# chris-chambers/deap

Hardware: AMD Instinct MI355X
Metric: GPop/s (node-evals×cases/s) symreg 64K pop×1M cases, 1/2/4/8 GPUs (higher is better)
Workload: dtype f64

## Files before the change

### deap_amd/_lib.py

```python
import ctypes
import os

import numpy as np

_HERE = os.path.dirname(os.path.abspath(__file__))
LIB_PATH = os.environ.get("DEAP_AMD_LIB") or os.path.join(_HERE, "libgpeval.so")

GPE_MACHINE_F = 0
GPE_MACHINE_B = 1
GPE_MODE_MSE = 0
GPE_MODE_HITS_BOOL = 1
GPE_MODE_HITS_BITS = 2
GPE_MODE_SSE_NUMPY = 3
GPE_MODE_SSE_SEQ = 4
GPE_PREC_F64 = 0
GPE_PREC_F32 = 1
GPE_NO_ERROR = 0xFFFFFFFFFFFFFFFF
GPE_ERR_VALUE = 1
GPE_ERR_OVERFLOW = 2
GPE_ERR_XINT_RANGE = 3
GPE_XINT_WORDS = 34
GPE_FLAG_NONFINITE_TERM = 1
GPE_FLAG_NAN_TERM = 2
GPE_FLAG_INF_TERM = 4
# ... 628 lines not shown
                         "asm_deep_P", "asm_deep_groups",
                         "asm_deep_waves_per_block", "redo_exact_cpp",
                         "asm_typed", "asm_typed_P", "asm_typed_groups",
                         "typed_const"),
                        list(g)))

    LAUNCHES = ("asm_fast", "asm_deep", "typed", "cpp_fast", "cpp_deep",
                "fasm", "dasm")

    def trig_classes(self, picked=False):
        if picked:
            g = (ctypes.c_int64 * len(TRIG_PICKED))()
            self._check(self.lib.gpe_last_trig_picked(self.h, g),
                        "gpe_last_trig_picked")
            return dict(zip(TRIG_PICKED, (int(v) for v in g)))
        g = (ctypes.c_int64 * 3)()
        self._check(self.lib.gpe_last_trig_classes(self.h, g),
                    "gpe_last_trig_classes")
        return dict(zip(TRIG_CLASSES, (int(v) for v in g)))

    def launch_shape(self, which):
        if isinstance(which, str):
            which = self.LAUNCHES.index(which)
        g = (ctypes.c_int64 * 12)()
        self._check(self.lib.gpe_last_launch_shape(self.h, int(which), g, 12),
                    "gpe_last_launch_shape")
        return dict(zip(("programs", "P", "wpb", "waves", "n_slots", "K",
                         "sdepth", "n_tiles", "tiles_per_group", "groups",
                         "dbuf", "lds_bytes"), list(g)))
```

### deap_amd/csrc/asm_kernels.h

```cpp
#pragma once
namespace {

struct AsmTask {
  const uint32_t* code;
  const uint32_t* start;
  const int32_t* slot_prog;
  int64_t n_slots;
  int P;
  const double* X;
  int nv;
  const double* terms;
  int nt;
  int64_t n_cases;
  int64_t n_tiles;
  int tiles_per_group;
  double* part;
  double* case_out;
  unsigned long long* first_err;
  uint32_t* flags;
  uint32_t* redo;
  uint32_t* redo_count;
  uint64_t* redo_list;
  uint32_t redo_list_cap;
  const double* cst;
  const float* cst32;
  int diag;
  uint32_t redo_hi;
  uint32_t* base_probe;
  int dbuf;
};

constexpr int kTrigLdsDoubles = asmcore::kTrigEntries * 2 + 4;
constexpr uint32_t kTrigLdsBytes = kTrigLdsDoubles * sizeof(double);
static_assert(kTrigLdsBytes % 16 == 0, "the X tile is read with 16-byte alignment");
constexpr int kCstTable = 16;

#if GP_ASM_LOOP
#define GP_CORE_LOOPED(CODE, PROBE, PROBE_OUT, J, NMINE, DONE, RHI, LEAN, VSTART,  \
                       VTS, VACC)                                             \
  asm volatile(GP_ASM_CORE                                                  \
               : GP_ASM_T_OUTPUTS, GP_ASM_VRED_OUTPUT, GP_ASM_VINF_OUTPUT,  \
                 [jio] "+s"(J)                                              \
               : [cst] "s"(cst), [xa] "v"(xa),                              \
                 [mg] "v"(asmcore::kAsmMagic), [ps2] "v"(asmcore::kAsmPs2), \
                 [pc2] "v"(asmcore::kAsmPc2), [one] "v"(0x3ff00000u),        \
                 [probe] "s"(PROBE), [probe_out] "s"(PROBE_OUT),            \
                 [code_lo] "s"((uint32_t)(CODE)),                           \
                 [code_hi] "s"((uint32_t)((uint64_t)(CODE) >> 32)),         \
                 [nmine] "s"(NMINE), [done] "s"(DONE), [rhi] "s"(RHI),      \
                 [lean] "s"(LEAN), [vstart] "v"(VSTART), [vts] "v"(VTS),    \
                 [vacc] "v"(VACC)                                           \
               : GP_ASM_CLOBBERS)
// ... 15 lines not shown
               : GP_ASM_CLOBBERS)
#define GP_CORE_LOOPED(CODE, PROBE, PROBE_OUT, J, NMINE, DONE, RHI, LEAN, VSTART,  \
                       VTS, VACC)                                             \
  __builtin_trap()
#endif

#define GP_CORE32(PC, PROBE, PROBE_OUT)                                     \
  asm volatile(GP_ASM_CORE32                                                \
               : GP_ASM_T_OUTPUTS32                                         \
               : [pc] "s"(PC), [cst] "s"(cst), [xa] "v"(xa),               \
                 [probe] "s"(PROBE), [probe_out] "s"(PROBE_OUT)             \
               : GP_ASM_CLOBBERS32)

#define GP_CORE_DEEP(PC, PROBE, PROBE_OUT)                                  \
  asm volatile(GP_ASM_CORE_DEEP                                             \
               : GP_ASM_T_OUTPUTS_DEEP, GP_ASM_VRED_OUTPUT_DEEP, GP_ASM_VINF_OUTPUT_DEEP                   \
               : [pc] "s"(PC), [cst] "s"(cst), [xa] "v"(xa),               \
                 [mg] "v"(asmcore::kAsmMagic), [ps2] "v"(asmcore::kAsmPs2), \
                 [pc2] "v"(asmcore::kAsmPc2), [one] "v"(0x3ff00000u),        \
                 [probe] "s"(PROBE),                                        \
                 [probe_out] "s"(PROBE_OUT)                                 \
               : GP_ASM_CLOBBERS_DEEP)

#if GP_ASM_LOOP_EXACT
#define GP_CORE_EXACT_LOOPED(CODE, PROBE, PROBE_OUT, J, NMINE, DONE, RHI, LEAN,   \
                             VSTART, VTS, VACC)                               \
  asm volatile(GP_ASM_CORE_EXACT                                            \
               : GP_ASM_T_OUTPUTS_EXACT, GP_ASM_VRED_OUTPUT_EXACT,          \
                 [jio] "+s"(J)                                              \
               : [cst] "s"(cst), [xa] "v"(xa),                              \
                 [mg] "v"(asmcore::kAsmMagic), [one] "v"(0x3ff00000u),      \
                 GP_ASM_GLIBC_INPUTS_EXACT, [probe] "s"(PROBE),             \
                 [probe_out] "s"(PROBE_OUT),                                \
                 [code_lo] "s"((uint32_t)(CODE)),                           \
                 [code_hi] "s"((uint32_t)((uint64_t)(CODE) >> 32)),         \
                 [nmine] "s"(NMINE), [done] "s"(DONE), [rhi] "s"(RHI),      \
                 [lean] "s"(LEAN), [vstart] "v"(VSTART), [vts] "v"(VTS),    \
                 [vacc] "v"(VACC)                                           \
               : GP_ASM_CLOBBERS_EXACT)
#define GP_CORE_EXACT(PC, PROBE, PROBE_OUT)                                 \
  do {                                                                      \
    uint32_t j_one_ = 0;                                                    \
    GP_CORE_EXACT_LOOPED((PC), (PROBE), (PROBE_OUT), j_one_, 1u, 0u, ~0u, 0u, \
                         0u, 0u, 0u);                                       \
  } while (0)
#else
#define GP_CORE_EXACT(PC, PROBE, PROBE_OUT)                                 \
  asm volatile(GP_ASM_CORE_EXACT                                            \
               : GP_ASM_T_OUTPUTS_EXACT, GP_ASM_VRED_OUTPUT_EXACT           \
               : [pc] "s"(PC), [cst] "s"(cst), [xa] "v"(xa),               \
                 [mg] "v"(asmcore::kAsmMagic), [one] "v"(0x3ff00000u),      \
                 GP_ASM_GLIBC_INPUTS_EXACT, [probe] "s"(PROBE),             \
                 [probe_out] "s"(PROBE_OUT)                                 \
               : GP_ASM_CLOBBERS_EXACT)
#define GP_CORE_EXACT_LOOPED(CODE, PROBE, PROBE_OUT, J, NMINE, DONE, RHI, LEAN,   \
                             VSTART, VTS, VACC)                               \
  __builtin_trap()
#endif

#define GP_CORE_EXACT_DEEP(PC, PROBE, PROBE_OUT)                            \
  asm volatile(GP_ASM_CORE_EXACT_DEEP                                       \
               : GP_ASM_T_OUTPUTS_EXACT_DEEP, GP_ASM_VRED_OUTPUT_EXACT_DEEP \
               : [pc] "s"(PC), [cst] "s"(cst), [xa] "v"(xa),               \
                 [mg] "v"(asmcore::kAsmMagic), [one] "v"(0x3ff00000u),      \
                 GP_ASM_GLIBC_INPUTS_EXACT_DEEP, [probe] "s"(PROBE),        \
                 [probe_out] "s"(PROBE_OUT)                                 \
               : GP_ASM_CLOBBERS_EXACT_DEEP)

#define GP_CORE32_DEEP(PC, PROBE, PROBE_OUT)                                \
  asm volatile(GP_ASM_CORE32_DEEP                                           \
               : GP_ASM_T_OUTPUTS32_DEEP                                    \
               : [pc] "s"(PC), [cst] "s"(cst), [xa] "v"(xa),               \
                 [probe] "s"(PROBE), [probe_out] "s"(PROBE_OUT)             \
               : GP_ASM_CLOBBERS32_DEEP)

__global__ __launch_bounds__(64) void f_probe_asm(const double* cst,
                                                  uint32_t* table) {
  double T[asmcore::K];
  uint32_t vred, vinf;
// ... 207 lines not shown
  Task st{};
  st.X = a.X;
  st.nv = a.nv;
  st.terms = a.terms;
  st.nt = a.nt;
  st.n_cases = a.n_cases;
  const uint32_t ncol = (uint32_t)(a.nv + a.nt);
  auto dma_tile = [&](int64_t t, uint32_t b) {
    const uint32_t w = (uint32_t)__builtin_amdgcn_readfirstlane(wave);
    for (uint32_t col = w; col < ncol; col += (uint32_t)nwaves) {
      const double* src = (col < (uint32_t)a.nv)
                              ? a.X + (int64_t)col * a.n_cases
                              : a.terms + (int64_t)(col - a.nv) * a.n_cases;
      src += t * (K * 64) + 2 * lane;
      const uint32_t dst = kTab + b * tile_bytes + col * (uint32_t)(K * 64 * sizeof(double));
      uint32_t keep;
      asm volatile("s_mov_b32 %0, m0\n\ts_mov_b32 m0, %2\n\ts_nop 0\n\t"
                   "global_load_lds_dwordx4 %1, off\n\ts_mov_b32 m0, %0"
                   : "=&s"(keep) : "v"(src), "s"(dst) : "memory");
    }
  };
  auto tile_full = [&](int64_t t) { return (t + 1) * (K * 64) <= a.n_cases; };
  bool staged = false;
  uint32_t gflag = 0;
  for (int64_t t = t0; t < t1; ++t) {
    if (a.diag & 16) {
      uint32_t sink;
      asm volatile(".rept 40\n\tv_readlane_b32 %0, %1, 5\n\t.endr" : "=s"(sink) : "v"(lane));
    }
    if constexpr (!F32 && !EXACT) {
      done_mask |= (uint32_t)__builtin_amdgcn_ballot_w64(gflag != 0);
      gflag = my_prog >= 0 ? __hip_atomic_load(&a.redo[my_prog], __ATOMIC_RELAXED,
                                                __HIP_MEMORY_SCOPE_AGENT)
                           : 0u;
    }
    if (dbuf) {
      const uint32_t b = (uint32_t)((t - t0) & 1);
      xs = xs0 + b * tile_elems;
      ts = xs + a.nv * K * 64;
      xa = kTab + b * tile_bytes + (uint32_t)lane * (uint32_t)sizeof(R);
      vts = xa + (uint32_t)(a.nv * K * 64 * (int)sizeof(R));
      if (!staged) {
        __syncthreads();
        f_stage<K>(st, xs, t, nthreads);
        __syncthreads();
      }
      staged = t + 1 < t1 && tile_full(t + 1);
      if (staged) dma_tile(t + 1, b ^ 1u);
    } else if (!(a.diag & 2) || t == t0) {
      if (!(a.diag & 4) || t == t0) __syncthreads();
      if (!(a.diag & 8) || t == t0) f_stage<K>(st, xs, t, nthreads);
      if (!(a.diag & 4) || t == t0) __syncthreads();
    }
    const int64_t case0 = t * (K * 64) + lane;
    const bool full = (t + 1) * (K * 64) <= a.n_cases;
    auto finish = [&](int j, int prog, R (&T)[K], uint32_t (&vcase)[F32 ? K : 1],
                      uint32_t vbits, bool redo_lane) {
      if (a.diag & 1) {
        if (T[0] == R(12345) && T[1] == R(54321)) acc[lane] = vcase[0];
        return;
      }
      if (__builtin_amdgcn_ballot_w64(redo_lane)) {
        if (lane == 0) {
          const uint32_t i = atomicAdd(a.redo_count, 1u);
          if ((F32 || EXACT) && i < a.redo_list_cap)
            a.redo_list[i] = ((uint64_t)(uint32_t)prog << 32) | (uint64_t)(uint32_t)t;
          atomicOr(&a.redo[prog], 1u);
        }
        if (!F32 && !EXACT) done_mask |= 1u << j;
        return;
      }
      double hi = acc[(2 * j) * 64 + lane], lo = acc[(2 * j + 1) * 64 + lane];
      if (lean && full) {
        double s = hi, l = lo;
#pragma unroll
        for (int k = 0; k < K; ++k) {
          const double dlt = (double)T[k] - (double)ts[k * 64 + lane];
// ... 31 lines not shown
          double s, e;
          two_sum(hi, sq, s, e);
          hi = s;
          lo = lo + e;
          if (a.case_out) a.case_out[(size_t)prog * a.n_cases + c] = sq;
        }
      }
      acc[(2 * j) * 64 + lane] = hi;
      acc[(2 * j + 1) * 64 + lane] = lo;
      if (err != ~0ull) atomicMin(&a.first_err[prog], err);
      if (__builtin_amdgcn_ballot_w64(flag != 0)) {
        for (int m = 32; m >= 1; m >>= 1) flag |= __shfl_xor(flag, m, 64);
        if (lane == 0) atomicOr(&a.flags[prog], flag);
      }
    };
    if constexpr (LOOP) {
      const uint32_t lean_full = (uint32_t)__builtin_amdgcn_readfirstlane(lean && full ? 1 : 0);
      const uint32_t probe =
          (uint32_t)__builtin_amdgcn_readfirstlane(a.base_probe != nullptr ? 1 : 0);
      uint32_t* probe_out = a.base_probe;
      const double* cst = a.cst;
      const uint64_t code = (uint64_t)a.code;
      uint32_t jn = 0;
#pragma nounroll
      for (;;) {
        uint32_t jx = jn;
        const uint32_t done = (uint32_t)__builtin_amdgcn_readfirstlane(done_mask);
        R T[K];
        uint32_t vred, vinf = 0;
        if constexpr (EXACT) {
          GP_CORE_EXACT_LOOPED(code, probe, probe_out, jx, (uint32_t)n_mine, done,
                               a.redo_hi, lean_full, my_start, vts, vacc);
        } else {
          GP_CORE_LOOPED(code, probe, probe_out, jx, (uint32_t)n_mine, done, a.redo_hi,
                         lean_full, my_start, vts, vacc);
        }
        if (probe || jx >= (uint32_t)n_mine) break;
        const int prog = __builtin_amdgcn_readlane(my_prog, jx);
        uint32_t vcase[1] = {vred};
        finish((int)jx, prog, T, vcase, vinf, vred >= a.redo_hi);
        jn = jx + 1;
      }
    } else {
#pragma nounroll
      for (int j = 0; j < n_mine; ++j) {
        if (done_mask & (1u << j)) continue;
        const int prog = __builtin_amdgcn_readlane(my_prog, j);
        const uint32_t w0 = __builtin_amdgcn_readlane(my_start, j);
        const uint64_t pc = (uint64_t)(a.code + w0);
        const uint32_t probe =
            (uint32_t)__builtin_amdgcn_readfirstlane(a.base_probe != nullptr ? 1 : 0);
        uint32_t* probe_out = a.base_probe;
        R T[K];
        uint32_t vcase[F32 ? K : 1];
        uint32_t vbits = 0;
        bool redo_lane;
        if constexpr (F32) {
          const float* cst = a.cst32;
          uint32_t* vred = vcase;
          if constexpr (DEEP) {
            GP_CORE32_DEEP(pc, probe, probe_out);
          } else {
            GP_CORE32(pc, probe, probe_out);
          }
// ... 221 lines not shown
```

### deap_amd/csrc/ctx.h

```cpp
#pragma once

struct Launch {
  std::vector<int32_t> slot_prog;
  int32_t* d_slot_prog = nullptr;
  int64_t n_slots = 0;
  int P = 1;
  int sdepth = 1;
  int wpb = kWaves;
  int64_t n_tiles = 0;
  int groups = 0;
  int tiles_per_group = 0;
  int64_t waves = 0;
  double* d_part = nullptr;
  size_t part_cap = 0;
  size_t slot_cap = 0;
  int64_t programs = 0;
  int K = 0;
  bool dbuf = false;
  size_t lds = 0;
  char* h_pin = nullptr;
  size_t h_pin_cap = 0;
};


constexpr int32_t kNpAdd = -1, kNpZero = -2;
constexpr int64_t kNpChunk = 8192, kNpBlock = 128;
constexpr int kNpStack = 64;

HD double np_leaf(const double* x, int64_t n) {
  if (n < 8) {
    double res = -0.0;
    for (int64_t i = 0; i < n; ++i) res = res + x[i];
    return res;
  }
  double r[8];
  for (int j = 0; j < 8; ++j) r[j] = x[j];
  int64_t i = 8;
  for (; i < n - (n % 8); i += 8)
    for (int j = 0; j < 8; ++j) r[j] = r[j] + x[i + j];
  double res = ((r[0] + r[1]) + (r[2] + r[3])) + ((r[4] + r[5]) + (r[6] + r[7]));
  for (; i < n; ++i) res = res + x[i];
// ... 201 lines not shown
  uint64_t* d_pair_sorted = nullptr;
  size_t pair_sorted_cap = 0;
  int64_t* d_pair_off = nullptr;
  size_t pair_off_cap = 0;
  uint32_t* d_pair_nruns = nullptr;
  size_t pair_nruns_cap = 0;
  char* d_sort_tmp = nullptr;
  size_t sort_tmp_cap = 0;
  int use_asm = 1;
  int asm_pmax = 8;
  int typed_pmax = 64;
  int typed_waves = 8;
  int64_t target_blocks = 8192;
  int64_t asm_target_blocks = 65536;
  int64_t xasm_target_blocks = 65536;
  int64_t typed_target_blocks = 32768;
  int64_t min_group_tiles = 0;
  int trig_w = 14;
  int div_w = 5;
  int deal_mix = 0;
  int asm_waves = 8;
  int asm_lds_kb = 80;
  int asm_dbuf = 1;
  int lw_interleave = 1;
  int neg_fold = 1;
  int exact_all = 1;
  int trig_ranges = 2;
  std::vector<double> col_bnd;
  double* d_col_bnd = nullptr;
  unsigned long long* d_trig_cls = nullptr;
  int64_t trig_classes[8] = {0, 0, 0, 0, 0, 0, 0, 0};
  std::vector<uint32_t> debug_redo_or;
  int asm_deep_waves = 4;
  int f_waves = 8;
  int b_lanes = 1;
  int diag = 0;
  uint32_t redo_hi = (uint32_t)asmcore::LIM_HI;
  uint32_t redo_hi_deep = (uint32_t)(0x3ff + 20) << 20;
  Launch fast, deep, fasm, dasm, tasm, redo_fast, redo_deep, redo_xasm, redo_xasm_deep;
  bool last_exact_all = false;
  std::vector<int32_t> pl_fa, pl_da, pl_ta, pl_fc, pl_dc, pl_order;
  std::vector<uint32_t> pl_kc;
  uint32_t* d_kc = nullptr;
  size_t kc_cap = 0;
  int64_t n_kc = 0;
  int64_t label_true = 0;
// ... 108 lines not shown
```

### deap_amd/csrc/gen_asm.py

```python
#!/usr/bin/env python3
import os
import re
import sys

HERE = os.path.dirname(os.path.abspath(__file__))

FAMS = ["add", "sub", "rsub", "mul", "div", "rdiv", "ndiv", "nrdiv"]
FAMS_TYPED = ["add", "sub", "rsub", "mul", "div", "rdiv", "lt", "gt", "eq",
              "and", "or"]
WINDOW = 16
MAGIC = "0x1.8p+52"
TINY_HI = 0x3e500000
LIM_HI = 0x42700000
FAST_EXP = int(os.environ.get("GEN_ASM_FAST_EXP", "14"))
FAST_HI = (0x3ff + FAST_EXP) << 20
SGPR_CONSTS = ["INV", "S1", "FAST", "NS2", "Ps0", "Ps1", "Pc1", "C1"]
TAB_ENTRIES = 768
TAB_BYTES = 16 * TAB_ENTRIES
COS_OFF = 16 * 128
SPLIT_TAB = os.environ.get("GEN_ASM_SPLIT_TAB", "0") == "1"
GLIBC_TAB_BYTES = 440 * 8
GLIBC_BRANRED_BYTES = GLIBC_TAB_BYTES
GLIBC_BRANRED_CONSTS = ["SPLIT", "BBIG1", "BMP2", "PAD"]
GLIBC_COSTAB = GLIBC_TAB_BYTES + 8 * (4 + 75 + 1)
GLIBC_LDS_BYTES = GLIBC_COSTAB + GLIBC_TAB_BYTES
GLIBC_SGPR = ["HPINV", "MP1", "MP2", "PP3", "PP4", "BIG", "HP0", "HP1",
              "SN3", "CS4", "CS2", "S4", "S3", "S2", "S1", "C0126"]
GLIBC_VGPR = ["SN5", "CS6", "S5", "HP1_LO", "HP1_HI"]
BRANRED_HI = 0x419921FB
GLIBC2 = os.environ.get("GEN_ASM_GLIBC2", "1") == "1"
GLIBC3 = GLIBC2 and os.environ.get("GEN_ASM_GLIBC3", "1") == "1"
ILP = os.environ.get("GEN_ASM_EXPERIMENT") == "ilp"
GLIBC4 = GLIBC3 and not ILP and os.environ.get("GEN_ASM_GLIBC4", "1") == "1"
GLIBC_SPLIT_S = 7 * 256
GLIBC_T0855 = 0x3feb6000
OOL = os.environ.get("GEN_ASM_OOL", "1") == "1"
TRIG_DROP = os.environ.get("GEN_ASM_TRIG_DROP", "wait")
EARLY = os.environ.get("GEN_ASM_EARLY", "1") == "1"
SALU = os.environ.get("GEN_ASM_SALU", "1") == "1"
if GLIBC4:
    GLIBC_BRANRED_BYTES = 3 * GLIBC_SPLIT_S
    GLIBC_COSTAB = None
    GLIBC_LDS_BYTES = GLIBC_BRANRED_BYTES + 8 * (4 + 75 + 1)


class Gen(object):
    def __init__(self, K, D, NV, TB0=32, SB=None, exact=False, trig_group=0,
                 loop=False, typed=False):
        if SB is None:
            SB = 40 if exact else 56
        self.K, self.D, self.NV = K, D, NV
        self.exact = exact
        self.loop = loop
        self.typed = typed
        self.fams = FAMS_TYPED if typed else FAMS
        self.trig_group = trig_group or int(os.environ.get("GEN_ASM_TRIG_GROUP", "0"))
        self.rskip = exact and os.environ.get("GEN_ASM_RSKIP", "1") == "1"
        self.read2 = os.environ.get("GEN_ASM_READ2", "0") == "1"
        pr = os.environ.get("GEN_ASM_PRIO", "tiered_late")
        self.prio = None if typed or (exact and not loop) else \
            {"trig_low": (1, 0), "trig_high": (0, 1), "tiered": (2, 0, 1),
             "tiered_late": (2, 0, 1), "tiered_late_div0": (2, 0, 0),
             "tiered_late_div2": (2, 0), "tiered_late1": (2, 1, 1)}.get(pr)
        self.prio_late = self.prio is not None and pr.startswith("tiered_late")
        self.align = int(os.environ.get("GEN_ASM_ALIGN", "0"))
        assert (NV * K - 1) * 512 < 65536, "NV * K too large for LDS offsets"
        self.TB0 = TB0
        self.RB = TB0 + 2 * K
        self.VRED = self.RB + 2 * K * D
        self.VINF = self.VRED + 1
        self.POOL0 = self.VRED + 2
        assert self.POOL0 % 2 == 0
        self.OB = self.POOL0 + 10
        self.vmax = self.OB + 2 * K
        assert SB % 4 == 0
        self.SB = SB
# ... 1725 lines not shown
                if key not in where:
                    kind = 1 if v in singles else 4 if v in quads else 2
                    where[key] = get(kind)
                name(names, v, where[key])
            if multi:
                for v in dying:
                    put(v, where.pop(kk(k, v)))
            for line in t.split("\n"):
                if line in ("<OOL>", "<MAIN>"):
                    self._in_ool = line == "<OOL>"
                    continue
                self.e(line.format(**names) if "{" in line else line)
            for v in d:
                key = kk(k, v)
                if key in where and last[key] == idx:
                    put(v, where.pop(key))
        self.use_v(nxt[0] - 1)

    def loop_next(self):
        W, NX = self.WIN, self.NXT
        self.e("s_nop 4")
        self.label(".Lnext_")
        self.e("s_cmp_ge_u32 s%d, %%[nmine]" % self.SJ)
        self.e("s_cbranch_scc1 .Lend_%=")
        self.e("s_bitcmp1_b32 %%[done], s%d" % self.SJ)
        self.e("s_cbranch_scc1 .Lskip_%=")
        if self.prefetch:
            self.e("s_cmp_eq_u32 s%d, s%d" % (self.SPF, self.SJ))
            self.e("s_cbranch_scc1 .Lhave_%=")
        self.load_first_window(self.SJ)
        self.label(".Lhave_")
        if self.prefetch:
            self.e("s_mov_b32 s%d, -1" % self.SPF)
        self.e("v_mov_b32_e32 v%d, 0" % self.VRED)
        if not self.exact:
            self.e("v_mov_b32_e32 v%d, 0" % self.VINF)
        self.e("s_mov_b32 m0, 0")
        self.e("s_waitcnt lgkmcnt(0)")
        self.e("s_nop 0")
        self.dispatch_head()
        self.dispatch_tail()
        self.label(".Lskip_")
        if self.prefetch:
            self.e("s_waitcnt lgkmcnt(0)")
        self.e("s_add_u32 s%d, s%d, 1" % (self.SJ, self.SJ))
        self.e("s_branch .Lnext_%=")

    def load_first_window(self, sj):
        W, NX = self.WIN, self.NXT
        self.e("v_readlane_b32 s%d, %%[vstart], s%d" % (NX, sj))
        self.e("s_nop 4")
        self.e("s_lshl_b32 s%d, s%d, 2" % (NX, NX))
        self.e("s_add_u32 s%d, %%[code_lo], s%d" % (self.PTR, NX))
        self.e("s_addc_u32 s%d, %%[code_hi], 0" % (self.PTR + 1))
        self.e("s_load_dwordx16 s[%d:%d], %s, 0x0"
               % (W, W + 15, self.sp(self.PTR)))

    def loop_end(self):
        K, P = self.K, self.p
        self.e("s_cmp_eq_u32 %[lean], 0")
        self.e("s_cbranch_scc1 .Lend_%=")
        self.e("v_cmp_le_u32_e64 vcc, %%[rhi], v%d" % self.VRED)
        self.e("s_and_b64 vcc, exec, vcc")
        self.e("s_cbranch_vccnz .Lend_%=")
        if not self.exact:
            self.e("v_cmp_ne_u32_e32 vcc, 0, v%d" % self.VINF)
            self.e("s_and_b64 vcc, exec, vcc")
            self.e("s_cbranch_vccnz .Lend_%=")
# ... 375 lines not shown
                    break
                seen.add((i, clean))
                l = lines[i]
                if l.startswith(".Lh_"):
                    break
                m = re.match(r"s_\w+ exec, (.*)$", l)
                if m:
                    clean = l.startswith("s_mov_b64") and m.group(1).strip() == saved
                if l.startswith("v_cmpx"):
                    clean = False
                if l.startswith("s_setpc_b64"):
                    assert clean, "EXEC not restored before %r (line %d)" % (l, i)
                    break
                m = re.match(r"s_(cbranch_\w+|branch) (\S+)$", l)
                if m:
                    assert m.group(2) in lab, m.group(2)
                    if m.group(1) == "branch":
                        i = lab[m.group(2)]
                        continue
                    stack.append((lab[m.group(2)], clean))
                i += 1


def trig_data():
    import json
    with open(os.path.join(HERE, "trig_table.json")) as fh:
        return json.load(fh)


def trig_const_block():
    d = trig_data()
    ps, pc, cc = d["Ps"], d["Pc"], d["C"]
    assert float.fromhex(pc[0]) == -0.5
    ns2 = (-float.fromhex(d["S2"])).hex()
    cpp = [d["INV"], d["S1"], "0x0p+0", ns2, "0x1p+40", "0x1p-26",
           "0x1p+%d" % FAST_EXP, ps[0], ps[1], ps[2], pc[1], pc[2], cc[0], cc[1], cc[2],
           MAGIC]

    val = {"INV": d["INV"], "S1": d["S1"], "FAST": "0x1p+%d" % FAST_EXP, "NS2": ns2,
           "Ps0": ps[0], "Ps1": ps[1], "Pc1": pc[1], "C1": cc[0]}
    core = [val[n] for n in SGPR_CONSTS]
    lds_tail = [ps[2], pc[2], cc[1], cc[2]]
    return cpp, core, lds_tail


def emit(K, D, NV, suffix="", out_dir=HERE, trig_group=0):
    exact = suffix in ("_exact", "_exact_deep")
    typed = suffix == "_typed"
    loop = typed or (suffix in ("", "_exact") and
                     os.environ.get("GEN_ASM_LOOP", "1") == "1")
    tb0 = int(os.environ.get("GEN_ASM_TB0", "32")) if suffix == "" else 32
    g = Gen(K, D, NV, TB0=tb0, exact=exact, loop=loop, typed=typed,
            trig_group=trig_group).build()
    g.vmax += int(os.environ.get("GEN_ASM_PAD_VGPRS", "0")) if not suffix else 0
    S = suffix.upper()
    lay = g.layout()
    body = g.lines
    if exact:
        check_exec(body, g.sp(g.SMASK))
    inc = os.path.join(out_dir, "gp_asm_core%s.inc" % suffix)
    with open(inc, "w") as fh:
        fh.write("// GENERATED by gen_asm.py (K=%d, D=%d, NV=%d) — do not edit\n"
                 % (K, D, NV))
        if suffix in ("", "_exact"):
            fh.write("#define GP_ASM_LOOP%s %d\n" % (suffix.upper(),
                                                     1 if g.loop else 0))
        fh.write("#define GP_ASM_CORE%s \\\n" % S)
        for l in body:
            fh.write('  "%s\\n" \\\n' % l)
        fh.write('  ""\n')
        outs = set(range(g.TB0, g.TB0 + 2 * K)) | {g.VRED}
        if not exact:
            outs.add(g.VINF)
        clob = ['"v%d"' % r for r in range(g.TB0, g.vmax) if r not in outs]
        clob += ['"s%d"' % r for r in range(g.SB, g.SMAX + 1)]
        clob += ['"vcc"', '"scc"', '"memory"']
        fh.write("#define GP_ASM_CLOBBERS%s %s\n" % (S, ", ".join(clob)))
        fh.write("#define GP_ASM_T_OUTPUTS%s %s\n" % (S, ", ".join(
            '[T%d] "=&{v[%d:%d]}"(T[%d])' % (k, g.T(k), g.T(k) + 1, k)
            for k in range(K))))
        fh.write('#define GP_ASM_VRED_OUTPUT%s [vred] "=&{v%d}"(vred)\n'
                 % (S, g.VRED))
        if not exact:
            fh.write('#define GP_ASM_VINF_OUTPUT%s [vinf] "=&{v%d}"(vinf)\n'
                     % (S, g.VINF))
        else:
            ins = []
            for n in GLIBC_VGPR:
                if GLIBC3 and n.startswith("HP1_"):
# ... 75 lines not shown
```

### deap_amd/csrc/gpeval.hip

```cpp
#include <dlfcn.h>
#include <hip/hip_runtime.h>
#include <hipcub/hipcub.hpp>
#include <array>

#include "host_pool.h"
#include <rccl/rccl.h>
#include <stdint.h>
#include <string.h>

#include <algorithm>
#include <chrono>
#include <cstdio>
#include <cstdlib>
#include <numeric>
#include <string>
#include <thread>
#include <type_traits>
#include <vector>

#include "../../include/gpeval.h"
#include "lower_core.h"
#include "trig_ranges.h"
#include "gp_asm_core.inc"
#include "gp_asm_core32.inc"
// ... 1412 lines not shown
    ctx->min_group_tiles = atol(env);
  if ((env = getenv("GPE_XASM_TARGET_BLOCKS")) && atol(env) >= 64)
    ctx->xasm_target_blocks = atol(env);
  if ((env = getenv("GPE_TRIG_W")) && atoi(env) >= 0 && atoi(env) <= 1000)
    ctx->trig_w = atoi(env);
  if ((env = getenv("GPE_DEAL_MIX"))) ctx->deal_mix = atoi(env);
  if ((env = getenv("GPE_DIV_W")) && atoi(env) >= 0 && atoi(env) <= 1000)
    ctx->div_w = atoi(env);
  if ((env = getenv("GPE_DIAG"))) ctx->diag = atoi(env);
  if ((env = getenv("GPE_EXACT_ALL"))) ctx->exact_all = atoi(env) != 0;
  if ((env = getenv("GPE_TRIG_RANGES")))
    ctx->trig_ranges = atoi(env) <= 0 ? trig_ranges::kOff
                       : atoi(env) == 1 ? trig_ranges::kBase : trig_ranges::kAll;
  if ((env = getenv("GPE_REDO_EXP")) && atoi(env) >= 14 && atoi(env) <= 40)
    ctx->redo_hi = (uint32_t)(0x3ff + atoi(env)) << 20;
  if ((env = getenv("GPE_REDO_EXP_DEEP")) && atoi(env) >= 14 && atoi(env) <= 40)
    ctx->redo_hi_deep = (uint32_t)(0x3ff + atoi(env)) << 20;
  if ((env = getenv("GPE_ASM_WAVES")) && atoi(env) >= 2 &&
      atoi(env) * 64 <= kAsmMaxBlock)
    ctx->asm_waves = atoi(env);
  if ((env = getenv("GPE_ASM_LDS_KB")) && atoi(env) >= 16 && atoi(env) <= 160)
    ctx->asm_lds_kb = atoi(env);
  if ((env = getenv("GPE_ASM_DBUF"))) ctx->asm_dbuf = atoi(env) != 0;
  if ((env = getenv("GPE_LOWER_IL"))) ctx->lw_interleave = atoi(env) != 0;
  if ((env = getenv("GPE_NEG_PEEPHOLE"))) ctx->neg_fold = atoi(env) != 0;
  if ((env = getenv("GPE_ASM_DEEP_WAVES")) && (atoi(env) == 4 || atoi(env) == 8))
    ctx->asm_deep_waves = atoi(env);
  if ((env = getenv("GPE_F_WAVES")) && (atoi(env) == 4 || atoi(env) == 8))
    ctx->f_waves = atoi(env);
  if ((env = getenv("GPE_B_LANES"))) ctx->b_lanes = atoi(env) != 0;
  if ((env = getenv("GPE_TYPED_ASM"))) ctx->use_typed = atoi(env) != 0;
  if ((env = getenv("GPE_TYPED_PMAX")) && atoi(env) >= 1 && atoi(env) <= 64)
    ctx->typed_pmax = atoi(env);
  if ((env = getenv("GPE_TYPED_WAVES")) && atoi(env) >= 1 && atoi(env) <= 16)
    ctx->typed_waves = atoi(env);
  auto init = [&]() -> int {
    HIPCHK(hipSetDevice(device));
    HIPCHK(hipStreamCreateWithFlags(&ctx->stream, hipStreamNonBlocking));
    for (auto& e : ctx->ev) HIPCHK(hipEventCreate(&e));
    for (auto& e : ctx->ev_redo) HIPCHK(hipEventCreate(&e));
    HIPCHK(hipEventCreateWithFlags(&ctx->ev_lw, hipEventDisableTiming));
    hipDeviceProp_t prop;
    HIPCHK(hipGetDeviceProperties(&prop, device));
    ctx->cu = prop.multiProcessorCount;
    ctx->clock_khz = prop.clockRate;
    snprintf(ctx->name, sizeof(ctx->name), "%s", prop.gcnArchName);
// ... 1738 lines not shown
  g[14] = ctx->tasm.P;
  g[15] = ctx->tasm.groups;
  g[16] = ctx->planned_mode == GPE_MODE_HITS_BOOL ? ctx->n_kc : 0;
  std::copy(g, g + std::min(n, GPE_GEOMETRY_FIELDS), o);
  return 0;
}

int gpe_last_launch_shape(const gpe_ctx* ctx, int which, int64_t* o, int n) {
  if (!ctx || !o || n < 0) return GPE_E_INVALID;
  const bool x = ctx->last_exact_all;
  const Launch* L = nullptr;
  switch (which) {
    case GPE_LAUNCH_ASM_FAST: L = x ? &ctx->redo_xasm : &ctx->fasm; break;
    case GPE_LAUNCH_ASM_DEEP: L = x ? &ctx->redo_xasm_deep : &ctx->dasm; break;
    case GPE_LAUNCH_TYPED: L = &ctx->tasm; break;
    case GPE_LAUNCH_CPP_FAST: L = &ctx->fast; break;
    case GPE_LAUNCH_CPP_DEEP: L = &ctx->deep; break;
    case GPE_LAUNCH_FASM: L = &ctx->fasm; break;
    case GPE_LAUNCH_DASM: L = &ctx->dasm; break;
    default: return GPE_E_INVALID;
  }
  const int64_t g[GPE_LAUNCH_SHAPE_FIELDS] = {
      L->programs, L->P, L->wpb, L->waves, L->n_slots, L->K, L->sdepth, L->n_tiles,
      L->tiles_per_group, L->groups, L->dbuf ? 1 : 0, (int64_t)L->lds};
  std::copy(g, g + std::min(n, GPE_LAUNCH_SHAPE_FIELDS), o);
  return 0;
}

}
```

### deap_amd/csrc/planner.h

```cpp
#pragma once
namespace {

int fast_k(const gpe_ctx* ctx) {
  return ctx->prec == GPE_PREC_F32 ? kFK32 : kFK;
}

int cases_per_tile(const gpe_ctx* ctx, bool deep, int asm_k) {
  if (ctx->machine == GPE_MACHINE_F)
    return asm_k ? 64 * asm_k : deep ? 64 : 64 * fast_k(ctx);
  return 64;
}

int asm_core_k(const gpe_ctx* ctx, bool deep_core, bool exact, bool typed) {
  if (typed) return asmcore_typed::K;
  if (ctx->prec == GPE_PREC_F32 && !exact) return asmcore32::K;
  if (exact) return asmcore_exact::K;
  return deep_core ? asmcore_deep::K : asmcore::K;
}

size_t lds_bytes(const gpe_ctx* ctx, bool deep, int sdepth = 0, int wpb = kWaves) {
  if (ctx->machine == GPE_MACHINE_F) {
    const int K = deep ? 1 : fast_k(ctx);
    const int D = sdepth > 0 ? sdepth : deep ? kDeepDepth : kFastDepth;
    const size_t el = ctx->prec == GPE_PREC_F32 ? sizeof(float) : sizeof(double);
// ... 271 lines not shown
  a.nt = ctx->nt;
  a.n_cases = ctx->n_cases;
  a.n_tiles = L.n_tiles;
  a.tiles_per_group = L.tiles_per_group;
  a.part = L.d_part;
  a.case_out = ctx->case_on ? ctx->d_case_out : nullptr;
  a.first_err = err;
  a.flags = flags;
  a.redo = ctx->d_redo;
  a.redo_count = ctx->d_redo_count;
  a.redo_list = ctx->d_redo_list;
  a.redo_list_cap = ctx->redo_list_cap;
  a.cst = ctx->d_cst;
  a.cst32 = ctx->d_cst32;
  a.diag = ctx->diag;
  a.redo_hi = deep_core ? std::min(ctx->redo_hi, ctx->redo_hi_deep) : ctx->redo_hi;
  if (exact) {
    a.redo = ctx->d_redo2;
    a.redo_count = ctx->d_redo2_count;
    a.redo_hi = asmcore_exact::EXACT_REDO_HI;
    a.cst = ctx->d_cst_exact;
  }
  a.dbuf = L.dbuf ? 1 : 0;
  const size_t lds = lds_bytes_asm(ctx, L.P, L.wpb, L.K, L.dbuf, exact);
  L.lds = lds;
  const bool f32 = ctx->prec == GPE_PREC_F32;
  auto kern = exact ? (deep_core ? f_eval_asm<false, true, true> : f_eval_asm<false, false, true>)
              : deep_core ? (f32 ? f_eval_asm<true, true> : f_eval_asm<false, true>)
                          : (f32 ? f_eval_asm<true, false> : f_eval_asm<false, false>);
  HIPCHK(hipFuncSetAttribute((const void*)kern,
                             hipFuncAttributeMaxDynamicSharedMemorySize, (int)lds));
  dim3 grid((unsigned)L.groups, (unsigned)(L.waves / L.wpb));
  hipLaunchKernelGGL(kern, grid, dim3(64 * L.wpb), lds, ctx->stream, a);
  HIPCHK(hipGetLastError());
  return 0;
}

int launch_asm_typed(gpe_ctx* ctx, Launch& L) {
  if (L.n_slots == 0) return 0;
  AsmTask a{};
  a.code = ctx->d_acode_t;
  a.start = ctx->d_astart_t;
  a.slot_prog = L.d_slot_prog;
  a.n_slots = L.n_slots;
  a.P = L.P;
  a.X = (const double*)ctx->d_X;
// ... 66 lines not shown
```

### include/gpeval.h

```cpp
#ifndef GPEVAL_H
#define GPEVAL_H

#include <stddef.h>
#include <stdbool.h>
#include <stdint.h>

#ifdef __cplusplus
extern "C" {
#endif

typedef struct gpe_ctx gpe_ctx;

#define GPE_MACHINE_F 0
#define GPE_MACHINE_B 1

#define GPE_MODE_MSE 0
#define GPE_MODE_HITS_BOOL 1
#define GPE_MODE_HITS_BITS 2
#define GPE_MODE_SSE_NUMPY 3
#define GPE_MODE_SSE_SEQ 4

#define GPE_PREC_F64 0
#define GPE_PREC_F32 1

// ... 110 lines not shown

int gpe_run_gathered(gpe_ctx* ctx, int mode, int64_t width,
                     const uint8_t* tags, double* out_hi, double* out_lo,
                     uint64_t* out_err, uint32_t* out_flags);

int gpe_last_timing(const gpe_ctx* ctx, float* ms);

int gpe_last_comm_timing(gpe_ctx* ctx, float* ms);

int gpe_debug_bounded_wait(double timeout_s, int64_t busy_polls, char* msg, size_t n);

int gpe_last_geometry(const gpe_ctx* ctx, int64_t* out8);

#define GPE_GEOMETRY_FIELDS 17
int gpe_last_geometry_ex(const gpe_ctx* ctx, int64_t* out, int n);

#define GPE_LAUNCH_ASM_FAST 0
#define GPE_LAUNCH_ASM_DEEP 1
#define GPE_LAUNCH_TYPED 2
#define GPE_LAUNCH_CPP_FAST 3
#define GPE_LAUNCH_CPP_DEEP 4
#define GPE_LAUNCH_FASM 5
#define GPE_LAUNCH_DASM 6
#define GPE_LAUNCH_SHAPE_FIELDS 12
int gpe_last_launch_shape(const gpe_ctx* ctx, int which, int64_t* out, int n);

int gpe_debug_translate(const uint32_t* code, int64_t n_words,
                        const int64_t* off, int64_t n_prog,
                        const int32_t* depth, int nv, const uint32_t* table,
                        int n_table, uint32_t* out, int64_t out_cap,
                        int64_t* starts, int64_t* n_out);

int gpe_debug_translate_ranges(const uint32_t* code, int64_t n_words,
                               const int64_t* off, int64_t n_prog,
                               const int32_t* depth, int nv, const uint32_t* table,
                               int n_table, uint32_t* out, int64_t out_cap,
                               int64_t* starts, int64_t* n_out, const double* lo,
                               const double* hi);

int gpe_debug_trig_classes(const uint32_t* code, int64_t n_words, const double* lo,
                           const double* hi, int nv, int32_t* out, int64_t cap);

int gpe_last_trig_classes(const gpe_ctx* ctx, int64_t* out);

int gpe_debug_translate_mode(const uint32_t* code, int64_t n_words,
                                const int64_t* off, int64_t n_prog,
                                const int32_t* depth, int nv, const uint32_t* table,
// ... 38 lines not shown
```

Measured before the change: 3913.

## Keep exact asm core resident across case tiles with in-asm LDS DMA

Adds a tile loop inside the generated exact-mode assembly core. When all programs on a tile finish, the core stays inside the asm block. It advances to the next tile, flips the double-buffer offsets, and issues global_load_lds DMA for the following tile itself. This avoids leaving the asm block, re-staging and re-entering per tile, and is meant to overlap the next tile's loads with evaluation. It adds a barrier inside the asm plus a static checker for the control flow. It is enabled by default only under narrow conditions (K=2, dbuf, lean, one term column, no case output).

```diff
diff --git a/deap_amd/_lib.py b/deap_amd/_lib.py
--- a/deap_amd/_lib.py
+++ b/deap_amd/_lib.py
@@ -674,9 +674,9 @@
     def launch_shape(self, which):
         if isinstance(which, str):
             which = self.LAUNCHES.index(which)
-        g = (ctypes.c_int64 * 12)()
-        self._check(self.lib.gpe_last_launch_shape(self.h, int(which), g, 12),
+        g = (ctypes.c_int64 * 13)()
+        self._check(self.lib.gpe_last_launch_shape(self.h, int(which), g, 13),
                     "gpe_last_launch_shape")
         return dict(zip(("programs", "P", "wpb", "waves", "n_slots", "K",
                          "sdepth", "n_tiles", "tiles_per_group", "groups",
-                         "dbuf", "lds_bytes"), list(g)))
+                         "dbuf", "lds_bytes", "tile_loop"), list(g)))
diff --git a/deap_amd/csrc/asm_kernels.h b/deap_amd/csrc/asm_kernels.h
--- a/deap_amd/csrc/asm_kernels.h
+++ b/deap_amd/csrc/asm_kernels.h
@@ -28,6 +28,7 @@
   uint32_t redo_hi;
   uint32_t* base_probe;
   int dbuf;
+  int tile_loop;
 };
 
 constexpr int kTrigLdsDoubles = asmcore::kTrigEntries * 2 + 4;
@@ -89,26 +90,33 @@
                  [probe_out] "s"(PROBE_OUT)                                 \
                : GP_ASM_CLOBBERS_DEEP)
 
+#ifndef GP_ASM_TILE_LOOP_EXACT
+#define GP_ASM_TILE_LOOP_EXACT 0
+#endif
 #if GP_ASM_LOOP_EXACT
 #define GP_CORE_EXACT_LOOPED(CODE, PROBE, PROBE_OUT, J, NMINE, DONE, RHI, LEAN,   \
-                             VSTART, VTS, VACC)                               \
+                             VSTART, XA, VTS, VACC, TIO, TEND, BFLIP, DLO, DHI,   \
+                             DDST)                                            \
   asm volatile(GP_ASM_CORE_EXACT                                            \
                : GP_ASM_T_OUTPUTS_EXACT, GP_ASM_VRED_OUTPUT_EXACT,          \
-                 [jio] "+s"(J)                                              \
-               : [cst] "s"(cst), [xa] "v"(xa),                              \
+                 [jio] "+s"(J), [tio] "+&s"(TIO), [bflip] "+&s"(BFLIP),     \
+                 [xa] "+&v"(XA), [vts] "+&v"(VTS)                           \
+               : [cst] "s"(cst),                                            \
                  [mg] "v"(asmcore::kAsmMagic), [one] "v"(0x3ff00000u),      \
                  GP_ASM_GLIBC_INPUTS_EXACT, [probe] "s"(PROBE),             \
                  [probe_out] "s"(PROBE_OUT),                                \
                  [code_lo] "s"((uint32_t)(CODE)),                           \
                  [code_hi] "s"((uint32_t)((uint64_t)(CODE) >> 32)),         \
                  [nmine] "s"(NMINE), [done] "s"(DONE), [rhi] "s"(RHI),      \
-                 [lean] "s"(LEAN), [vstart] "v"(VSTART), [vts] "v"(VTS),    \
-                 [vacc] "v"(VACC)                                           \
+                 [lean] "s"(LEAN), [vstart] "v"(VSTART),                    \
+                 [vacc] "v"(VACC), [tend] "s"(TEND), [dlo] "v"(DLO),        \
+                 [dhi] "v"(DHI), [ddst] "v"(DDST)                           \
                : GP_ASM_CLOBBERS_EXACT)
 #define GP_CORE_EXACT(PC, PROBE, PROBE_OUT)                                 \
   do {                                                                      \
-    uint32_t j_one_ = 0;                                                    \
+    uint32_t j_one_ = 0, t_one_ = 0, flip_one_ = 0, xa_one_ = xa, vts_one_ = 0; \
     GP_CORE_EXACT_LOOPED((PC), (PROBE), (PROBE_OUT), j_one_, 1u, 0u, ~0u, 0u, \
+                         0u, xa_one_, vts_one_, 0u, t_one_, 0u, flip_one_,  \
                          0u, 0u, 0u);                                       \
   } while (0)
 #else
@@ -121,7 +129,8 @@
                  [probe_out] "s"(PROBE_OUT)                                 \
                : GP_ASM_CLOBBERS_EXACT)
 #define GP_CORE_EXACT_LOOPED(CODE, PROBE, PROBE_OUT, J, NMINE, DONE, RHI, LEAN,   \
-                             VSTART, VTS, VACC)                               \
+                             VSTART, XA, VTS, VACC, TIO, TEND, BFLIP, DLO, DHI,   \
+                             DDST)                                            \
   __builtin_trap()
 #endif
 
@@ -375,6 +384,21 @@
   };
   auto tile_full = [&](int64_t t) { return (t + 1) * (K * 64) <= a.n_cases; };
   bool staged = false;
+  constexpr bool kResident = LOOP && EXACT && GP_ASM_TILE_LOOP_EXACT;
+  const bool resident = kResident && dbuf && lean && a.tile_loop && a.n_tiles < (1ll << 31);
+  const int64_t t_full = min(t1, a.n_cases / (K * 64));
+  uint32_t dma_lo = 0, dma_hi = 0, dma_dst = 0;
+  if (resident) {
+    const uint32_t col = (uint32_t)wave + (uint32_t)lane * (uint32_t)nwaves;
+    if (col < ncol) {
+      const double* src = (col < (uint32_t)a.nv)
+                              ? a.X + (int64_t)col * a.n_cases
+                              : a.terms + (int64_t)(col - a.nv) * a.n_cases;
+      dma_lo = (uint32_t)(uint64_t)src;
+      dma_hi = (uint32_t)((uint64_t)src >> 32);
+      dma_dst = kTab + col * (uint32_t)(K * 64 * sizeof(double));
+    }
+  }
   uint32_t gflag = 0;
   for (int64_t t = t0; t < t1; ++t) {
     if (a.diag & 16) {
@@ -405,7 +429,7 @@
       if (!(a.diag & 8) || t == t0) f_stage<K>(st, xs, t, nthreads);
       if (!(a.diag & 4) || t == t0) __syncthreads();
     }
-    const int64_t case0 = t * (K * 64) + lane;
+    int64_t case0 = t * (K * 64) + lane;
     const bool full = (t + 1) * (K * 64) <= a.n_cases;
     auto finish = [&](int j, int prog, R (&T)[K], uint32_t (&vcase)[F32 ? K : 1],
                       uint32_t vbits, bool redo_lane) {
@@ -483,6 +507,10 @@
       const double* cst = a.cst;
       const uint64_t code = (uint64_t)a.code;
       uint32_t jn = 0;
+      [[maybe_unused]] uint32_t tio = (uint32_t)t;
+      [[maybe_unused]] const uint32_t tend = !kResident ? 0u :
+          (uint32_t)__builtin_amdgcn_readfirstlane(resident && full ? (uint32_t)t_full : 0u);
+      [[maybe_unused]] uint32_t bflip = ((t - t0) & 1) ? 0u - tile_bytes : tile_bytes;
 #pragma nounroll
       for (;;) {
         uint32_t jx = jn;
@@ -491,7 +519,16 @@
         uint32_t vred, vinf = 0;
         if constexpr (EXACT) {
           GP_CORE_EXACT_LOOPED(code, probe, probe_out, jx, (uint32_t)n_mine, done,
-                               a.redo_hi, lean_full, my_start, vts, vacc);
+                               a.redo_hi, lean_full, my_start, xa, vts, vacc, tio, tend,
+                               bflip, dma_lo, dma_hi, dma_dst);
+          if constexpr (kResident) {
+            if (tio != (uint32_t)t) {
+              t = (int64_t)tio;
+              xs = xs0 + ((t - t0) & 1) * tile_elems;
+              ts = xs + a.nv * K * 64;
+              case0 = t * (K * 64) + lane;
+            }
+          }
         } else {
           GP_CORE_LOOPED(code, probe, probe_out, jx, (uint32_t)n_mine, done, a.redo_hi,
                          lean_full, my_start, vts, vacc);
@@ -501,6 +538,9 @@
         uint32_t vcase[1] = {vred};
         finish((int)jx, prog, T, vcase, vinf, vred >= a.redo_hi);
         jn = jx + 1;
+      }
+      if constexpr (kResident) {
+        if (tend) staged = false;
       }
     } else {
 #pragma nounroll
diff --git a/deap_amd/csrc/ctx.h b/deap_amd/csrc/ctx.h
--- a/deap_amd/csrc/ctx.h
+++ b/deap_amd/csrc/ctx.h
@@ -17,6 +17,7 @@
   int64_t programs = 0;
   int K = 0;
   bool dbuf = false;
+  bool resident = false;
   size_t lds = 0;
   char* h_pin = nullptr;
   size_t h_pin_cap = 0;
@@ -264,6 +265,7 @@
   int asm_waves = 8;
   int asm_lds_kb = 80;
   int asm_dbuf = 1;
+  int tile_loop = 1;
   int lw_interleave = 1;
   int neg_fold = 1;
   int exact_all = 1;
diff --git a/deap_amd/csrc/gen_asm.py b/deap_amd/csrc/gen_asm.py
--- a/deap_amd/csrc/gen_asm.py
+++ b/deap_amd/csrc/gen_asm.py
@@ -46,12 +46,14 @@
 
 class Gen(object):
     def __init__(self, K, D, NV, TB0=32, SB=None, exact=False, trig_group=0,
-                 loop=False, typed=False):
+                 loop=False, typed=False, tile_loop=False):
         if SB is None:
             SB = 40 if exact else 56
         self.K, self.D, self.NV = K, D, NV
         self.exact = exact
         self.loop = loop
+        assert not tile_loop or (loop and exact)
+        self.tile_loop = tile_loop
         self.typed = typed
         self.fams = FAMS_TYPED if typed else FAMS
         self.trig_group = trig_group or int(os.environ.get("GEN_ASM_TRIG_GROUP", "0"))
@@ -1823,7 +1825,7 @@
         self.e("s_nop 4")
         self.label(".Lnext_")
         self.e("s_cmp_ge_u32 s%d, %%[nmine]" % self.SJ)
-        self.e("s_cbranch_scc1 .Lend_%=")
+        self.e("s_cbranch_scc1 %s" % (".Ltile_%=" if self.tile_loop else ".Lend_%="))
         self.e("s_bitcmp1_b32 %%[done], s%d" % self.SJ)
         self.e("s_cbranch_scc1 .Lskip_%=")
         if self.prefetch:
@@ -1845,6 +1847,50 @@
         if self.prefetch:
             self.e("s_waitcnt lgkmcnt(0)")
         self.e("s_add_u32 s%d, s%d, 1" % (self.SJ, self.SJ))
+        self.e("s_branch .Lnext_%=")
+        if self.tile_loop:
+            self.tile_next()
+
+    def tile_next(self):
+        assert self.K == 2
+        W, NX = self.WIN, self.NXT
+        VL = self.POOL0
+        self.label(".Ltile_")
+        self.e("s_add_u32 s%d, %%[tio], 1" % NX)
+        self.e("s_cmp_lt_u32 s%d, %%[tend]" % NX)
+        self.e("s_cbranch_scc0 .Lend_%=")
+        self.e("s_waitcnt vmcnt(0)")
+        self.e("s_barrier")
+        self.e("s_mov_b32 %%[tio], s%d" % NX)
+        self.e("v_add_u32_e32 %[xa], %[bflip], %[xa]")
+        self.e("v_add_u32_e32 %[vts], %[bflip], %[vts]")
+        self.e("s_sub_u32 %[bflip], 0, %[bflip]")
+        self.e("s_add_u32 s%d, s%d, 1" % (NX, NX))
+        self.e("s_cmp_lt_u32 s%d, %%[tend]" % NX)
+        self.e("s_cbranch_scc0 .Ltile_run_%=")
+        self.e("s_lshl_b32 s%d, s%d, 10" % (W + 2, NX))
+        self.e("s_lshr_b32 s%d, s%d, 22" % (W + 3, NX))
+        self.e("s_max_i32 s%d, %%[bflip], 0" % (W + 4))
+        self.e("s_mov_b32 s%d, 0" % (W + 5))
+        self.e("v_mbcnt_lo_u32_b32 v%d, -1, 0" % VL)
+        self.e("v_mbcnt_hi_u32_b32 v%d, -1, v%d" % (VL, VL))
+        self.e("v_lshlrev_b32_e32 v%d, 4, v%d" % (VL, VL))
+        self.label(".Ltile_dma_")
+        self.e("v_readlane_b32 s%d, %%[dlo], s%d" % (W, W + 5))
+        self.e("v_readlane_b32 s%d, %%[dhi], s%d" % (W + 1, W + 5))
+        self.e("v_readlane_b32 s%d, %%[ddst], s%d" % (W + 6, W + 5))
+        self.e("s_nop 4")
+        self.e("s_cmp_eq_u64 %s, 0" % self.sp(W))
+        self.e("s_cbranch_scc1 .Ltile_run_%=")
+        self.e("s_add_u32 s%d, s%d, s%d" % (W, W, W + 2))
+        self.e("s_addc_u32 s%d, s%d, s%d" % (W + 1, W + 1, W + 3))
+        self.e("s_add_u32 m0, s%d, s%d" % (W + 6, W + 4))
+        self.e("s_nop 0")
+        self.e("global_load_lds_dwordx4 v%d, %s" % (VL, self.sp(W)))
+        self.e("s_add_u32 s%d, s%d, 1" % (W + 5, W + 5))
+        self.e("s_branch .Ltile_dma_%=")
+        self.label(".Ltile_run_")
+        self.e("s_mov_b32 s%d, 0" % self.SJ)
         self.e("s_branch .Lnext_%=")
 
     def load_first_window(self, sj):
@@ -2266,6 +2312,58 @@
                 i += 1
 
 
+def check_tile_loop(lines, saved, sj):
+    lab = {l[:-1]: i for i, l in enumerate(lines)
+           if l.endswith(":") and not l.startswith(("s_", "v_"))}
+    assert sum(l.split()[0] == "s_barrier" for l in lines) == 1, "one s_barrier"
+    to_tile = [i for i, l in enumerate(lines) if l.endswith(" .Ltile_%=")]
+    assert len(to_tile) == 1 and lines[to_tile[0]].startswith("s_cbranch_scc1") \
+        and lines[to_tile[0] - 1].startswith("s_cmp_ge_u32 s%d, %%[nmine]" % sj) \
+        and lines[to_tile[0] - 2] == ".Lnext_%=:", ".Ltile is .Lnext's end of programs"
+    assert lines[lab[".Ltile_%="] - 1].startswith("s_branch"), "fall into .Ltile"
+    reset = "s_mov_b32 s%d, 0" % sj
+    resets = [i for i, l in enumerate(lines) if l == reset]
+    seen, ends = set(), set()
+    stack = [(lab[".Ltile_%="], 0, False)]
+    while stack:
+        i, nbar, zero = stack.pop()
+        while True:
+            assert i < len(lines), "ran off the core"
+            if (i, nbar, zero) in seen:
+                break
+            seen.add((i, nbar, zero))
+            l = lines[i]
+            if l == ".Lend_%=:":
+                assert nbar == 0 and not zero, "left the core after the barrier"
+                ends.add("end")
+                break
+            if l == ".Lnext_%=:":
+                assert nbar == 1 and zero, "tile change without its barrier / reset"
+                ends.add("next")
+                break
+            assert not l.startswith(".Lh_"), "fell into a handler"
+            assert not re.match(r"(s_\w+ exec,|v_cmpx|s_setpc)", l), \
+                "EXEC changed or a jump in the tile change: %r" % l
+            if l.split()[0] == "s_barrier":
+                nbar += 1
+            if l == reset:
+                assert nbar == 1
+                zero = True
+            m = re.match(r"s_(cbranch_\w+|branch) (\S+)$", l)
+            if m:
+                assert m.group(2) in lab, m.group(2)
+                if m.group(1) == "branch":
+                    i = lab[m.group(2)]
+                    continue
+                stack.append((lab[m.group(2)], nbar, zero))
+            i += 1
+    assert ends == {"end", "next"}, ends
+    tile = range(lab[".Ltile_%="], lab[".Ltile_run_%="] + 3)
+    assert all(i in tile for i in resets) and len(resets) == 1, "s%d reset elsewhere" % sj
+    a, b = lab[".Lnext_%="], lab[".Ltile_%="]
+    assert not any(re.match(r"(s_\w+ exec,|v_cmpx)", l) for l in lines[a:b]), "EXEC in .Lnext"
+
+
 def trig_data():
     import json
     with open(os.path.join(HERE, "trig_table.json")) as fh:
@@ -2294,14 +2392,18 @@
     loop = typed or (suffix in ("", "_exact") and
                      os.environ.get("GEN_ASM_LOOP", "1") == "1")
     tb0 = int(os.environ.get("GEN_ASM_TB0", "32")) if suffix == "" else 32
+    tile_loop = suffix == "_exact" and loop and \
+        os.environ.get("GEN_ASM_TILE_LOOP", "1") == "1"
     g = Gen(K, D, NV, TB0=tb0, exact=exact, loop=loop, typed=typed,
-            trig_group=trig_group).build()
+            trig_group=trig_group, tile_loop=tile_loop).build()
     g.vmax += int(os.environ.get("GEN_ASM_PAD_VGPRS", "0")) if not suffix else 0
     S = suffix.upper()
     lay = g.layout()
     body = g.lines
     if exact:
         check_exec(body, g.sp(g.SMASK))
+    if g.tile_loop:
+        check_tile_loop(body, g.sp(g.SMASK), g.SJ)
     inc = os.path.join(out_dir, "gp_asm_core%s.inc" % suffix)
     with open(inc, "w") as fh:
         fh.write("// GENERATED by gen_asm.py (K=%d, D=%d, NV=%d) — do not edit\n"
@@ -2309,6 +2411,8 @@
         if suffix in ("", "_exact"):
             fh.write("#define GP_ASM_LOOP%s %d\n" % (suffix.upper(),
                                                      1 if g.loop else 0))
+        if suffix == "_exact":
+            fh.write("#define GP_ASM_TILE_LOOP_EXACT %d\n" % (1 if g.tile_loop else 0))
         fh.write("#define GP_ASM_CORE%s \\\n" % S)
         for l in body:
             fh.write('  "%s\\n" \\\n' % l)
diff --git a/deap_amd/csrc/gpeval.hip b/deap_amd/csrc/gpeval.hip
--- a/deap_amd/csrc/gpeval.hip
+++ b/deap_amd/csrc/gpeval.hip
@@ -1458,6 +1458,7 @@
   if ((env = getenv("GPE_ASM_LDS_KB")) && atoi(env) >= 16 && atoi(env) <= 160)
     ctx->asm_lds_kb = atoi(env);
   if ((env = getenv("GPE_ASM_DBUF"))) ctx->asm_dbuf = atoi(env) != 0;
+  if ((env = getenv("GPE_TILE_LOOP"))) ctx->tile_loop = atoi(env) != 0;
   if ((env = getenv("GPE_LOWER_IL"))) ctx->lw_interleave = atoi(env) != 0;
   if ((env = getenv("GPE_NEG_PEEPHOLE"))) ctx->neg_fold = atoi(env) != 0;
   if ((env = getenv("GPE_ASM_DEEP_WAVES")) && (atoi(env) == 4 || atoi(env) == 8))
@@ -3242,7 +3243,8 @@
   }
   const int64_t g[GPE_LAUNCH_SHAPE_FIELDS] = {
       L->programs, L->P, L->wpb, L->waves, L->n_slots, L->K, L->sdepth, L->n_tiles,
-      L->tiles_per_group, L->groups, L->dbuf ? 1 : 0, (int64_t)L->lds};
+      L->tiles_per_group, L->groups, L->dbuf ? 1 : 0, (int64_t)L->lds,
+      L->resident ? 1 : 0};
   std::copy(g, g + std::min(n, GPE_LAUNCH_SHAPE_FIELDS), o);
   return 0;
 }
diff --git a/deap_amd/csrc/planner.h b/deap_amd/csrc/planner.h
--- a/deap_amd/csrc/planner.h
+++ b/deap_amd/csrc/planner.h
@@ -317,6 +317,10 @@
     a.cst = ctx->d_cst_exact;
   }
   a.dbuf = L.dbuf ? 1 : 0;
+  L.resident = exact && !deep_core && GP_ASM_LOOP_EXACT && GP_ASM_TILE_LOOP_EXACT &&
+               ctx->tile_loop && L.dbuf && L.K * 64 * sizeof(double) == 1024 &&
+               a.nt == 1 && a.case_out == nullptr && a.n_tiles < (1ll << 31);
+  a.tile_loop = L.resident ? 1 : 0;
   const size_t lds = lds_bytes_asm(ctx, L.P, L.wpb, L.K, L.dbuf, exact);
   L.lds = lds;
   const bool f32 = ctx->prec == GPE_PREC_F32;
diff --git a/include/gpeval.h b/include/gpeval.h
--- a/include/gpeval.h
+++ b/include/gpeval.h
@@ -156,7 +156,7 @@
 #define GPE_LAUNCH_CPP_DEEP 4
 #define GPE_LAUNCH_FASM 5
 #define GPE_LAUNCH_DASM 6
-#define GPE_LAUNCH_SHAPE_FIELDS 12
+#define GPE_LAUNCH_SHAPE_FIELDS 13
 int gpe_last_launch_shape(const gpe_ctx* ctx, int which, int64_t* out, int n);
 
 int gpe_debug_translate(const uint32_t* code, int64_t n_words,
```

New measurement: 4025, median of 6. 1.03x the previous value.
